# eggsbenedicto/DiffusionRenderer-ComfyUI

Hardware: AMD Instinct MI355X
Metric: denoising_steps_per_sec (higher is better)
Workload: dtype bf16; 1 GPU; inverse pass, 57f x 576 x 1024 clip: EDM Euler step = 1 DiT forward (D=4096, 28 blocks, 32 heads) over S=18432 tokens, guidance 0; parallelism=sp1 (token bands; self-attention exchange: none), weights=random-init (hash generator), 7.2e9 params bf16

## Files before the change

diffusionrenderer-comfyui_amd/csrc/attention.hip:

```cpp
#include <stdlib.h>
#include "drn_common.h"
#include "drn_launchers.h"
#include "mx_quant.h"

#ifndef ATT_EPI_LDS
#define ATT_EPI_LDS 1
#endif
#ifndef ATT_PRIO
#define ATT_PRIO 1
#endif
#ifndef ATT_ABL
#define ATT_ABL 0
#endif
#ifndef ATT_DIAG
#define ATT_DIAG 0
#endif
#ifndef ATT_DMA_IN_S
#define ATT_DMA_IN_S 0
#endif
static_assert(ATT_DMA_IN_S == 0, "ATT_DMA_IN_S > 0 reads clamped K/V rows for tile nt-2: fix S_REQ's offsets first");
#ifndef ATT_PTR
#define ATT_PTR 1
#endif
#ifndef ATT_TIE
// ... 490 lines not shown
    if (oq)
        attention_combine_kernel<true><<<grid, dim3(256), 0, st>>>(opart, mlpart, (bf16_t*)o, nsplit, batch, heads, Sq, ldo, bso,
                                                                   scale_log2e, (uint8_t*)oq, (uint8_t*)os, mx_bs);
    else
        attention_combine_kernel<false><<<grid, dim3(256), 0, st>>>(opart, mlpart, (bf16_t*)o, nsplit, batch, heads, Sq, ldo, bso,
                                                                    scale_log2e, nullptr, nullptr, 0);
}

#ifndef ATT_DEFAULT_SHAPE16
#define ATT_DEFAULT_SHAPE16 1
#endif
static int g_att16 = -1;
extern "C" void drn_attention_force_shape16(int on) { g_att16 = on; }

static bool attention_shape16() {
    static int env16 = -1;
    if (env16 < 0) {
        const char* e = getenv("DRN_ATT16");
        env16 = e ? (e[0] != '0') : ATT_DEFAULT_SHAPE16;
    }
    return (g_att16 >= 0 ? g_att16 : env16) != 0;
}

extern "C" int drn_attention_mx_available(void) { return attention_shape16() ? 1 : 0; }

static int attention_launch(const void* q, const void* k, const void* v, void* o, int batch, int heads, int64_t Sq, int64_t Sk,
                            int64_t ldq, int64_t ldk, int64_t ldv, int64_t ldo, int64_t bsq, int64_t bsk, int64_t bsv,
                            int64_t bso, float scale, int nsplit, void* workspace, void* stream, void* oq = nullptr,
                            void* os = nullptr) {
    DRN_CHECK_ARG(q && k && v && (o || oq) && batch > 0 && heads > 0 && Sq >= 0 && Sk > 0 && nsplit >= 1);
    DRN_CHECK_ARG(ldq % 8 == 0 && ldk % 8 == 0 && ldv % 8 == 0 && ldo % 8 == 0);
    DRN_CHECK_ARG(bsq % 8 == 0 && bsk % 8 == 0 && bsv % 8 == 0 && bso % 8 == 0);
    DRN_CHECK_ARG(((uintptr_t)q & 15) == 0 && ((uintptr_t)k & 15) == 0 && ((uintptr_t)v & 15) == 0 && ((uintptr_t)o & 15) == 0);
    DRN_CHECK_ARG(ldk > 0 && ldv > 0 && 64 * ldk * 2 < (1ll << 32) && 64 * ldv * 2 < (1ll << 32));
    AttnLaunch L;
    DRN_TRY(drn_attention_prologue(&L, oq, os, attention_shape16(), batch, heads, Sq, Sk, ldo, bso, scale, nsplit, workspace, QROWS, KVT));
    if (Sq == 0) return DRN_OK;
    hipStream_t st = (hipStream_t)stream;
    if (attention_shape16()) {
        drn_attention16_launch(q, k, v, o, heads, Sq, Sk, ldq, ldk, ldv, ldo, bsq, bsk, bsv, bso, L.scale_log2e, (int)L.nqb, L.total,
                               L.nsplit, L.kv_chunk, L.opart, L.mlpart, st, L.nsplit > 1 ? nullptr : oq, os, L.mx_bs);
    } else
    attention_fwd_kernel<<<dim3((unsigned)L.total, 1, 1), dim3(512), 0, st>>>(
        (const bf16_t*)q, (const bf16_t*)k, (const bf16_t*)v, (bf16_t*)o, heads, Sq, Sk, ldq, ldk, ldv, ldo, bsq, bsk,
        bsv, bso, L.scale_log2e, (int)L.nqb, (int)L.total, L.nsplit, L.kv_chunk, L.opart, L.mlpart);
    if (L.nsplit > 1)
        drn_attention_combine_launch(L.opart, L.mlpart, o, L.nsplit, batch, heads, Sq, ldo, bso, L.scale_log2e, oq, os, L.mx_bs, st);
    return drn_launch_status();
}

extern "C" int drn_attention_bf16(const void* q, const void* k, const void* v, void* o, int batch, int heads, int64_t Sq,
                                  int64_t Sk, int64_t ldq, int64_t ldk, int64_t ldv, int64_t ldo, int64_t bsq,
                                  int64_t bsk, int64_t bsv, int64_t bso, float scale, void* stream) {
    DRN_CHECK_ARG(o);
    return attention_launch(q, k, v, o, batch, heads, Sq, Sk, ldq, ldk, ldv, ldo, bsq, bsk, bsv, bso, scale, 1, nullptr, stream);
}

extern "C" int drn_attention_bf16_mx(const void* q, const void* k, const void* v, void* o, void* oq, void* os, int batch, int heads,
                                     int64_t Sq, int64_t Sk, int64_t ldq, int64_t ldk, int64_t ldv, int64_t ldo, int64_t bsq,
                                     int64_t bsk, int64_t bsv, int64_t bso, float scale, void* stream) {
    DRN_CHECK_ARG(oq && os);
    return attention_launch(q, k, v, o, batch, heads, Sq, Sk, ldq, ldk, ldv, ldo, bsq, bsk, bsv, bso, scale, 1, nullptr, stream, oq, os);
}

extern "C" int64_t drn_attention_splitkv_workspace_bytes(int batch, int heads, int64_t Sq, int nsplit) {
    return (int64_t)nsplit * batch * Sq * heads * (128 + 2) * (int64_t)sizeof(float);
}

extern "C" int drn_attention_splitkv_bf16(const void* q, const void* k, const void* v, void* o, int batch, int heads, int64_t Sq,
                                          int64_t Sk, int64_t ldq, int64_t ldk, int64_t ldv, int64_t ldo, int64_t bsq,
                                          int64_t bsk, int64_t bsv, int64_t bso, float scale, int nsplit, void* workspace,
                                          void* stream) {
    DRN_CHECK_ARG(o);
    return attention_launch(q, k, v, o, batch, heads, Sq, Sk, ldq, ldk, ldv, ldo, bsq, bsk, bsv, bso, scale, nsplit, workspace,
                            stream);
}

extern "C" int drn_attention_splitkv_bf16_mx(const void* q, const void* k, const void* v, void* o, void* oq, void* os, int batch,
                                             int heads, int64_t Sq, int64_t Sk, int64_t ldq, int64_t ldk, int64_t ldv, int64_t ldo,
                                             int64_t bsq, int64_t bsk, int64_t bsv, int64_t bso, float scale, int nsplit,
                                             void* workspace, void* stream) {
    DRN_CHECK_ARG(oq && os);
    return attention_launch(q, k, v, o, batch, heads, Sq, Sk, ldq, ldk, ldv, ldo, bsq, bsk, bsv, bso, scale, nsplit, workspace,
                            stream, oq, os);
}
```

diffusionrenderer-comfyui_amd/csrc/attention16.hip:

```cpp
#include "drn_common.h"
#include "drn_launchers.h"
#include "mx_quant.h"

#define QROWS 256
#define KVT 64
#define KBYTES (KVT * 256)
#define NKB 3
#define NVB 4
#ifndef RESCALE_THR
#define RESCALE_THR 6.0f
#endif

typedef const __attribute__((address_space(1))) void* gptr_t;
typedef __attribute__((address_space(3))) void* lptr_t;

template <bool MX>
__global__ __launch_bounds__(512, 2) void attention16_fwd_kernel(
    const bf16_t* __restrict__ Q, const bf16_t* __restrict__ Kp, const bf16_t* __restrict__ Vp, bf16_t* __restrict__ O,
    int heads, int64_t Sq, int64_t Sk_total, int64_t ldq, int64_t ldk, int64_t ldv, int64_t ldo, int64_t bsq, int64_t bsk,
    int64_t bsv, int64_t bso, float scale_log2e, int nqb, int total, int nsplit, int64_t kv_chunk,
    float* __restrict__ Opart, float* __restrict__ MLpart, uint8_t* __restrict__ OQ, uint8_t* __restrict__ OS, int64_t mx_bs) {
    __shared__ __attribute__((aligned(1024))) char smem[(NKB + NVB) * KBYTES];

    const int tid = threadIdx.x;
    const int lane = tid & 63;
    const int wave = __builtin_amdgcn_readfirstlane(tid >> 6);
    const int c = lane & 15, g = lane >> 4;

    int pid;
    {
        const int bid = blockIdx.x;
        const int q = total >> 3, r = total & 7, xcd = bid & 7;
        pid = (xcd < r ? xcd * (q + 1) : r * (q + 1) + (xcd - r) * q) + (bid >> 3);
    }
    const int qb = pid % nqb;
    const int rest = pid / nqb;
    const int split = rest % nsplit;
    const int bh = rest / nsplit;
    const int b = bh / heads, head = bh - b * heads;
    const int64_t q0 = (int64_t)qb * QROWS + wave * 32;
    const int64_t kv_begin = (int64_t)split * kv_chunk;
    const int64_t Sk = min(kv_chunk, Sk_total - kv_begin);

    const bf16_t* Qb = Q + b * bsq + (int64_t)head * 128;
    const bf16_t* Kb = Kp + b * bsk + kv_begin * ldk + (int64_t)head * 128;
    const bf16_t* Vb = Vp + b * bsv + kv_begin * ldv + (int64_t)head * 128;

    bf16x8_t qf[2][4];
#pragma unroll
    for (int qt = 0; qt < 2; ++qt) {
        int64_t qrow = q0 + 16 * qt + c;
        if (qrow > Sq - 1) qrow = Sq - 1;
        const bf16_t* qp = Qb + qrow * ldq + 8 * g;
#pragma unroll
        for (int ks = 0; ks < 4; ++ks) qf[qt][ks] = *reinterpret_cast<const bf16x8_t*>(qp + 32 * ks);
    }
#pragma unroll
    for (int qt = 0; qt < 2; ++qt)
#pragma unroll
        for (int ks = 0; ks < 4; ++ks) asm volatile("" : "+v"(qf[qt][ks]));

    int st_row[2], st_kc[2], st_vc[2];
#pragma unroll
    for (int i = 0; i < 2; ++i) {
        st_row[i] = 4 * (2 * wave + i) + (lane >> 4);
        const int cp = lane & 15;
        st_kc[i] = (cp ^ (st_row[i] & 15)) * 8;
        st_vc[i] = (cp ^ (((st_row[i] & 3) << 1) | (((st_row[i] >> 3) & 1) << 3))) * 8;
    }
    const int dma_off = wave * 2048;
    uint32_t kso[2], vso[2];
#pragma unroll
    for (int i = 0; i < 2; ++i) {
        kso[i] = 2u * (uint32_t)(st_row[i] * (int)ldk + st_kc[i]);
        vso[i] = 2u * (uint32_t)(st_row[i] * (int)ldv + st_vc[i]);
    }
    const int last_rows = (int)(Sk - (int64_t)((Sk - 1) / KVT) * KVT);
#define CLAMP_LAST_TILE()                                                                     \
    do {                                                                                      \
        _Pragma("unroll") for (int i = 0; i < 2; ++i) {                                       \
            const int r_ = min(st_row[i], last_rows - 1);                                     \
            kso[i] = 2u * (uint32_t)(r_ * (int)ldk + st_kc[i]);                               \
            vso[i] = 2u * (uint32_t)(r_ * (int)ldv + st_vc[i]);                               \
// ... 186 lines not shown
                pb[s_][qt] = cv.v;                                                            \
            }                                                                                 \
            if (!ATT16_LSUM_MFMA) l_run[qt] += ps[0] + ps[1];                                 \
        }                                                                                     \
    } while (0)

    const float thr_raw = RESCALE_THR / scale_log2e;
    float m_thr[2] = {-INFINITY, -INFINITY}, mcs[2] = {0.f, 0.f};
    const int nt = (int)((Sk + KVT - 1) / KVT);
    const int grp = wave >> 2;
    if (nt == 1 && last_rows < KVT) CLAMP_LAST_TILE();
    {
        const char* k0_ = reinterpret_cast<const char*>(Kb);
        const char* v0_ = reinterpret_cast<const char*>(Vb);
        DMA_PIECE_AT(0, k0_, v0_, 0, 0); DMA_PIECE_AT(1, k0_, v0_, 0, 0); DMA_PIECE_AT(2, k0_, v0_, 0, 0); DMA_PIECE_AT(3, k0_, v0_, 0, 0);
    }
    const int64_t ktile_bytes = (int64_t)KVT * ldk * 2, vtile_bytes = (int64_t)KVT * ldv * 2;
    if (nt > 1) {
        if (nt == 2 && last_rows < KVT) CLAMP_LAST_TILE();
        const char* k1_ = reinterpret_cast<const char*>(Kb) + ktile_bytes;
        const char* v1_ = reinterpret_cast<const char*>(Vb) + vtile_bytes;
        DMA_PIECE_AT(0, k1_, v1_, 1, 1); DMA_PIECE_AT(1, k1_, v1_, 1, 1); DMA_PIECE_AT(2, k1_, v1_, 1, 1); DMA_PIECE_AT(3, k1_, v1_, 1, 1);
    }
    DMA_WAIT(0);
    BARRIER();
    if (nt == 3 && last_rows < KVT) CLAMP_LAST_TILE();
    if (!ATT16_BAR1 && grp == 1) BARRIER();
    const char* kreq_p = reinterpret_cast<const char*>(Kb) + (int64_t)min(2, nt - 1) * ktile_bytes;
    const char* vreq_p = reinterpret_cast<const char*>(Vb) + (int64_t)min(2, nt - 1) * vtile_bytes;
    int kbuf = 0, vbuf = 0;
    int kreq = 2 % NKB, vreq = 2 % NVB;
#define REQ_PIECE_NOW(P)                                                                      \
    do {                                                                                      \
        if (!(ATT16_ABL & 4)) DMA_PIECE_AT(P, kreq_p, vreq_p, kreq, vreq);                    \
        FENCE();                                                                              \
    } while (0)
#define REQ_PIECE(P) do { if (!ATT16_DMA_IN_S) REQ_PIECE_NOW(P); } while (0)
#define AFTER_REQUESTS(T)                                                                     \
    do {                                                                                      \
        kreq = kreq == NKB - 1 ? 0 : kreq + 1;                                                \
        vreq = vreq == NVB - 1 ? 0 : vreq + 1;                                                \
        if ((T) + 3 == nt - 1 && last_rows < KVT) CLAMP_LAST_TILE();     \
        if (!(ATT16_ABL & 8) && (T) + 3 <= nt - 1) { kreq_p += ktile_bytes; vreq_p += vtile_bytes; }    \
    } while (0)
#define M_QK(T)                                                                               \
    do {                                                                                      \
// ... 112 lines not shown
            const int64_t qr = q0 + row;
            if (!MX) {
                if (qr < Sq) *reinterpret_cast<uint4*>(op + qr * ldo) = v;
            } else {
                uint32_t amax = max(max(mx_amax2(v.x), mx_amax2(v.y)), max(mx_amax2(v.z), mx_amax2(v.w)));
                amax = max(amax, (uint32_t)__shfl_xor((int)amax, 1, 64));
                amax = max(amax, (uint32_t)__shfl_xor((int)amax, 2, 64));
                const int e = mx_block_exp(amax);
                const float inv = mx_inv_scale(e);
                if (qr < Sq) {
                    const int64_t r = b * mx_bs + qr;
                    *reinterpret_cast<uint2*>(OQ + (r * heads + head) * 128 + oc * 8) = make_uint2(mx_pack4(v.x, v.y, inv), mx_pack4(v.z, v.w, inv));
                    if ((oc & 3) == 0) OS[(r * heads + head) * 4 + (oc >> 2)] = (uint8_t)(e + 127);
                    if (O) *reinterpret_cast<uint4*>(op + qr * ldo) = v;
                }
            }
        }
    }
}

void drn_attention16_launch(const void* q, const void* k, const void* v, void* o, int heads, int64_t Sq, int64_t Sk, int64_t ldq,
                            int64_t ldk, int64_t ldv, int64_t ldo, int64_t bsq, int64_t bsk, int64_t bsv, int64_t bso,
                            float scale_log2e, int nqb, int64_t total, int nsplit, int64_t kv_chunk, float* opart, float* mlpart,
                            hipStream_t st, void* oq, void* os, int64_t mx_bs) {
    if (oq)
        attention16_fwd_kernel<true><<<dim3((unsigned)total, 1, 1), dim3(512), 0, st>>>(
            (const bf16_t*)q, (const bf16_t*)k, (const bf16_t*)v, (bf16_t*)o, heads, Sq, Sk, ldq, ldk, ldv, ldo, bsq, bsk, bsv, bso,
            scale_log2e, nqb, (int)total, nsplit, kv_chunk, opart, mlpart, (uint8_t*)oq, (uint8_t*)os, mx_bs);
    else
        attention16_fwd_kernel<false><<<dim3((unsigned)total, 1, 1), dim3(512), 0, st>>>(
            (const bf16_t*)q, (const bf16_t*)k, (const bf16_t*)v, (bf16_t*)o, heads, Sq, Sk, ldq, ldk, ldv, ldo, bsq, bsk, bsv, bso,
            scale_log2e, nqb, (int)total, nsplit, kv_chunk, opart, mlpart, nullptr, nullptr, 0);
}
```

diffusionrenderer-comfyui_amd/csrc/dit_forward.hip:

```cpp
#include "drn_common.h"

static const int kCUs = 256;

static int64_t ceil_div(int64_t a, int64_t b) { return (a + b - 1) / b; }

static int pick_kv_splits(int64_t batch, int64_t heads, int64_t Sq, int64_t Sk, double* cost_out) {
    const int64_t blocks = batch * heads * ((Sq + 255) / 256);
    int best = 1;
    double best_cost = (double)ceil_div(blocks, kCUs);
    const int cand[3] = {2, 4, 8};
    for (int i = 0; i < 3; ++i) {
        const int n = cand[i];
        if (Sk / n < 512) break;
        const double cost = (double)ceil_div(blocks * n, kCUs) * (1.0 / n + 0.04) + 0.06;
        const double lim = (double)ceil_div(blocks, kCUs) * 0.93;
        if (cost < (best_cost < lim ? best_cost : lim)) {
            best = n;
            best_cost = cost;
        }
    }
    if (cost_out) *cost_out = best_cost;
    return best;
}

// ... 245 lines not shown
        }
        const int splits = drn_gemm_mxfp8_splitk_choice(clip_rows(M, rpb), N, K);
        Scope sc(timer(), 0, 2.0 * M * N * K, 1.03 * (M * K + N * K) + 2.0 * M * N * (l.residual ? 2 : 1), (hipStream_t)stream);
        if (c_is_mx) *c_is_mx = l.c_mx.q && l.epi == DRN_EPI_GELU && splits <= 1;
        if (c_is_mx && *c_is_mx) return drn_gemm_mxfp8_gelu_mx(A.q, A.s, l.w, l.sw, l.c_mx.q, l.c_mx.s, M, N, K, rpb, stream);
        if (splits == 0) return drn_gemm_mxfp8(A.q, A.s, l.w, l.sw, l.c, M, N, K, N, l.epi, l.gate, l.residual, ldr, rpb, stream);
        if (splits > 1 && defers(l)) {
            deferred = splits;
            deferred_gate = (const bf16_t*)l.gate;
            return drn_gemm_mxfp8_splitk_partials(A.q, A.s, l.w, l.sw, M, N, K, rpb, splits, a->gemm_ws, stream);
        }
        return drn_gemm_mxfp8_splitk(A.q, A.s, l.w, l.sw, l.c, M, N, K, N, l.epi, l.gate, l.residual, ldr, rpb, splits, a->gemm_ws, stream);
    }

    int linear(const Linear& l, bool* c_is_mx = nullptr) { return a->precision == 1 ? linear_mx(l, c_is_mx) : linear_bf16(l); }

    int self_attention(const drn_dit_sub* sb, bool mx_ops, bool o_mx) {
        const int64_t S = a->S, D = a->D, ld = 3 * D, bs = S * 3 * D;
        const int B = (int)a->B, heads = a->heads;
        const float sm_scale = (float)(1.0 / sqrt(128.0));
        bf16_t* q = (bf16_t*)a->QKV;
        bf16_t* k = q + D;
        bf16_t* v = q + 2 * D;
        uint8_t *mxa = nullptr, *kq = nullptr, *vt = nullptr, *ks = nullptr, *vs = nullptr;
        if (mx_ops) {
            mxa = (uint8_t*)a->mx_attn;
            kq = mxa + al[1], vt = mxa + al[2], ks = mxa + al[4], vs = mxa + al[5];
            DRN_TRY(drn_qk_norm_rope_mx(q, k, sb->qn, sb->kn, a->cos, a->sin, mxa + al[0], mxa + al[3], kq, ks, M, heads, ld, ld, S, 0,
                                        a->eps, 0, stream));
            DRN_TRY(drn_mx_quant_vt(v, vt, vs, B, heads, S, ld, bs, stream));
        } else {
            DRN_TRY(drn_qk_norm_rope(q, k, sb->qn, sb->kn, a->cos, a->sin, M, heads, ld, ld, S, 0, a->eps, stream));
        }
        Scope sc(timer(), 1, 4.0 * B * heads * S * S * 128, (mx_ops ? 1.0 : 2.0) * B * heads * 128 * (4.0 * S), (hipStream_t)stream);
        int64_t plan[6];
        const int n = drn_attention_plan(heads, S, S, plan);
        for (int p = 0; p < n; ++p) {
            const int64_t q0 = plan[3 * p], nq = plan[3 * p + 1] - q0;
            const int ns = (int)plan[3 * p + 2];
            bf16_t* o = o_mx ? nullptr : (bf16_t*)a->O + q0 * D;
            uint8_t* oq = o_mx ? (uint8_t*)a->AQ + q0 * D : nullptr;
            uint8_t* os = o_mx ? (uint8_t*)a->AS + q0 * (D / 32) : nullptr;
            if (mx_ops) {
                const uint8_t* qq = mxa + al[0] + q0 * D;
                const uint8_t* qs = mxa + al[3] + q0 * (D / 32);
                DRN_TRY(ns > 1 ? drn_attention_splitkv_mxfp8(qq, qs, kq, ks, vt, vs, o, oq, os, B, heads, nq, S, S, S, D, S * D, sm_scale, ns,
                                                             a->attn_ws, stream)
                               : drn_attention_mxfp8(qq, qs, kq, ks, vt, vs, o, oq, os, B, heads, nq, S, S, S, D, S * D, sm_scale, stream));
            } else if (o_mx) {
                DRN_TRY(ns > 1 ? drn_attention_splitkv_bf16_mx(q + q0 * ld, k, v, nullptr, oq, os, B, heads, nq, S, ld, ld, ld, D, bs, bs, bs,
                                                               S * D, sm_scale, ns, a->attn_ws, stream)
                               : drn_attention_bf16_mx(q + q0 * ld, k, v, nullptr, oq, os, B, heads, nq, S, ld, ld, ld, D, bs, bs, bs, S * D,
                                                       sm_scale, stream));
            } else {
                DRN_TRY(ns > 1 ? drn_attention_splitkv_bf16(q + q0 * ld, k, v, o, B, heads, nq, S, ld, ld, ld, D, bs, bs, bs, S * D, sm_scale,
                                                            ns, a->attn_ws, stream)
                               : drn_attention_bf16(q + q0 * ld, k, v, o, B, heads, nq, S, ld, ld, ld, D, bs, bs, bs, S * D, sm_scale, stream));
            }
        }
        return DRN_OK;
    }
};

int validate(const drn_dit_forward_args* a, int64_t al[8]) {
    DRN_CHECK_ARG(a && a->struct_bytes == (int64_t)sizeof(drn_dit_forward_args));
    DRN_CHECK_ARG(a->S > 0 && a->B > 0 && a->D > 0 && a->heads > 0 && a->D == (int64_t)a->heads * 128 && a->hidden > 0);
    DRN_CHECK_ARG(a->n_sub >= 0 && (a->n_sub == 0 || a->subs) && a->X && a->H && a->QKV && a->O && a->U && a->Y);
    DRN_CHECK_ARG(a->P && a->w_patch && a->w_final && a->final_shift && a->final_scale && a->shift && a->scale && a->gate);
    const int64_t S = a->S, B = a->B, D = a->D;
    DRN_CHECK_ARG(a->precision == 0 || a->precision == 1);
    int64_t need = drn_dit_forward_gemm_workspace_bytes(B, S, D, a->hidden, a->n_final, a->kpad);
// ... 88 lines not shown
```

diffusionrenderer-comfyui_amd/csrc/drn_launchers.h:

```cpp
#pragma once
#include "drn_common.h"

struct ConvGeom;

void drn_attention_combine_launch(const float* opart, const float* mlpart, void* o, int nsplit, int batch, int heads, int64_t Sq,
                                  int64_t ldo, int64_t bso, float scale_log2e, void* oq, void* os, int64_t mx_bs, hipStream_t st);
void drn_attention16_launch(const void* q, const void* k, const void* v, void* o, int heads, int64_t Sq, int64_t Sk, int64_t ldq,
                            int64_t ldk, int64_t ldv, int64_t ldo, int64_t bsq, int64_t bsk, int64_t bsv, int64_t bso,
                            float scale_log2e, int nqb, int64_t total, int nsplit, int64_t kv_chunk, float* opart, float* mlpart,
                            hipStream_t st, void* oq, void* os, int64_t mx_bs);

int drn_gemm256s_dispatch(const void* A, const void* W, void* C, int64_t M, int64_t N, int64_t K, int64_t lda, int64_t ldw,
                          int64_t ldc, int epilogue, const void* gate, const void* residual, int64_t ldr, int64_t rpb,
                          void* stream, const int64_t* blk);
int drn_gemm256s_partial(const void* A, const void* W, float* partial, int64_t M, int64_t N, int64_t K, int64_t lda, int64_t ldw,
                         int splits, void* stream, bool wring_ok);
int drn_gemm144_dispatch(const void* A, const void* W, void* C, int64_t M, int64_t N, int64_t K, int64_t lda, int64_t ldw,
                         int64_t ldc, int epilogue, const void* gate, const void* residual, int64_t ldr, int64_t rpb,
                         void* stream, const int64_t* blk);
int drn_gemm_tall_dispatch(const void* A, const void* W, void* C, float* partial, int64_t M, int64_t N, int64_t K, int64_t lda,
                           int64_t ldw, int64_t ldc, int epilogue, const void* gate, const void* residual, int64_t ldr,
                           int64_t rpb, int splits, void* stream);
int drn_gemm_splitk_reduce(const void* workspace, int splits, void* C, int64_t M, int64_t N, int64_t ldc, int epilogue,
                           const void* gate, const void* residual, int64_t ldr, int64_t rows_per_batch, void* stream);
int drn_gemm_mx_gelu_mx_launch(const void* A, const void* SA, const void* W, const void* SW, void* CQ, void* CS, int64_t M, int64_t N,
                               int64_t K, void* stream);

bool drn_conv256s_ok(const ConvGeom& g, int C, int N, int64_t ldc, int64_t ldr, bool has_residual, bool out_f32, const void* y,
                     const void* residual);
int drn_conv256s_launch(const void* x, const void* w, const void* bias, void* y, const void* residual, const ConvGeom& g, int C,
                        int N, int64_t ldw, int64_t ldc, int64_t ldr, void* stream);

struct AttnLaunch {
// ... 34 lines not shown
```

diffusionrenderer-comfyui_amd/dit_engine.py:

```python
import ctypes
import math
from typing import Dict, Optional

import torch

from . import native as N
from .host_tables import rope_cos_sin, timestep_sinusoid
from .parallel import ShardPlan, allgather_rows_, alltoall_bands_, alltoall_rows_, group_info, wait_exchange


PRECISIONS = ("bf16", "mxfp8")
ATTENTION_PRECISIONS = ("bf16", "mxfp8")


def _pad_cols(w: torch.Tensor, mult: int) -> torch.Tensor:
    n, k = w.shape
    kp = (k + mult - 1) // mult * mult
    if kp == k:
        return w.contiguous()
    out = torch.zeros((n, kp), dtype=w.dtype, device=w.device)
    out[:, :k] = w
    return out


# ... 430 lines not shown
                a.mx_fused = 1
                a.UQ, a.US = ws["uact"].data_ptr(), ws["uact"].data_ptr() + ws["uact_q_bytes"]
                a.u_act_bytes = ws["uact"].numel()
        if self._amx:
            a.attn_precision = 1
            a.mx_attn, a.mx_attn_bytes = ws["mx_attn"].data_ptr(), ws["mx_attn"].numel()
        return a

    def _fa_local(self, sb, hin, ws, cos, sin, gate, S, B, fusedmx):
        D = self.D
        X, O, QKV = ws["x"], ws["o"], ws["qkv"]
        self._lin(hin, sb["wqkv"], QKV, rows_per_batch=S)
        q, k, v = QKV[:, :D], QKV[:, D:2 * D], QKV[:, 2 * D:]
        amx = self._amx and N.attention_mxfp8_choice(self.heads, S)
        omx = (self._mx_view(ws["act"], ws["act_q_bytes"], X.shape[0], D)
               if fusedmx and (amx or N.attention_mx_available()) else None)
        if amx:
            qm, km, vt, vs = ws["mx_attn_views"]
            N.qk_norm_rope_mx(q, k, sb["qn"], sb["kn"], cos, sin, self.heads, tokens_per_batch=S,
                              write_bf16=self.trace is not None, out_q=qm, out_k=km)
            N.mx_quant_vt(QKV.view(B, S, 3 * D)[:, :, 2 * D:], self.heads, out=(vt, vs))
            oin = N.attention_mxfp8(qm, km, vt, vs, B, S, S, out=None if omx else O.view(B, S, D), out_mx=omx)
        else:
            N.qk_norm_rope(q, k, sb["qn"], sb["kn"], cos, sin, self.heads, tokens_per_batch=S)
            Q3 = QKV.view(B, S, 3 * D)
            oin = N.attention(Q3[:, :, :D], Q3[:, :, D:2 * D], Q3[:, :, 2 * D:], out=None if omx else O.view(B, S, D),
                              heads=self.heads, out_mx=omx)
        self._lin(oin if omx else O, sb["wo"], X, epilogue=N.EPI_GATE_RES, gate=gate, residual=X, rows_per_batch=S)

    def _mlp(self, sb, hin, ws, gate, rows, fusedmx):
        X, U = ws["x"], ws["u"]
        uin = U
        if fusedmx and N.mx_gemm_plan(X.shape[0], U.shape[1], self.D, rows) <= 1:
            uin = N.gemm_mxfp8(hin, sb["w1"], epilogue=N.EPI_GELU, rows_per_batch=rows,
                               out_mx=self._mx_view(ws["uact"], ws["uact_q_bytes"], X.shape[0], U.shape[1]))
        else:
            self._lin(hin, sb["w1"], U, epilogue=N.EPI_GELU, rows_per_batch=rows)
        self._lin(uin, sb["w2"], X, epilogue=N.EPI_GATE_RES, gate=gate, residual=X, rows_per_batch=rows)

    def _run(self, x, cond, mod, modf, addvec, Tp, Hp, Wp, plan):
        D = self.D
        S, rows, world = plan.S, plan.rows, plan.world
        B = x.shape[0]
        cos, sin = self.rope(Tp, Hp, Wp)
        ws = self._workspace(S, rows, B)
        X, Hb, O, Y = ws["x"], ws["h"], ws["o"], ws["y"]
        modB = modfB = gateB = None
        if B > 1:
            modB = mod[:, :2 * D].reshape(-1, 2, 1, D).expand(-1, 2, B, D).contiguous()
            modfB = modf.view(2, 1, D).expand(2, B, D).contiguous()
# ... 67 lines not shown
```

diffusionrenderer-comfyui_amd/native.py:

```python
import ctypes
import os
from ctypes import POINTER, Structure, c_char_p, c_double, c_float, c_int, c_int32, c_int64, c_void_p

import torch

_LIB = None
_LIB_NAME = "libdrn.so"

EPI_NONE, EPI_GELU, EPI_GATE_RES = 0, 1, 2
ACT_NONE, ACT_SILU = 0, 1

_P, _I, _L, _F = c_void_p, c_int, c_int64, c_float

SUB_FA, SUB_CA, SUB_MLP = 0, 1, 2


class DitSub(Structure):
    _fields_ = [("kind", c_int32), ("site", c_int32), ("ca_index", c_int32), ("reserved", c_int32),
                ("w_a", c_void_p), ("w_b", c_void_p), ("qn", c_void_p), ("kn", c_void_p),
                ("s_a", c_void_p), ("s_b", c_void_p)]


class DitForwardArgs(Structure):
    _fields_ = [("struct_bytes", c_int64), ("S", c_int64), ("B", c_int64), ("D", c_int64), ("hidden", c_int64),
# ... 28 lines not shown
    "drn_timer_read": [_P, _I, POINTER(c_int), POINTER(c_float), POINTER(c_double), POINTER(c_double)],
    "drn_abi_version": [],
    "drn_error_string": [_I],
    "drn_gemm_bf16": [_P, _P, _P, _L, _L, _L, _L, _L, _L, _I, _P, _P, _L, _L, _P],
    "drn_gemm_bf16_blocked": [_P, _P, _P, _L, _L, _L, _L, _L, _L, _I, _P, _P, _L, _L, _L, _L, _L, _L, _P],
    "drn_gemm_bf16_splitk": [_P, _P, _P, _L, _L, _L, _L, _L, _L, _I, _P, _P, _L, _L, _I, _P, _P],
    "drn_gemm_splitk_workspace_bytes": [_L, _L, _I],
    "drn_gemm_bf16_f32out": [_P, _P, _P, _L, _L, _L, _L, _L, _P],
    "drn_gemm_bf16_splitk_partials": [_P, _P, _L, _L, _L, _L, _L, _L, _I, _P, _P],
    "drn_splitk_gate_res_ln_modulate": [_P, _I, _P, _P, _P, _P, _P, _P, _L, _L, _L, _F, _P],
    "drn_gemm_splitk_choice": [_L, _L, _L],
    "drn_gemm_tile_choice": [_L, _L],
    "drn_gemm_force_tile": [_I],
    "drn_gemm_force_res_prefetch": [_I],
    "drn_gemm_tall_force_shape": [_I],
    "drn_mx_quant_bf16": [_P, _L, _L, _L, _P, _P, _P],
    "drn_mx_quant_calls": [_I],
    "drn_gemm_mxfp8_gelu_mx": [_P, _P, _P, _P, _P, _P, _L, _L, _L, _L, _P],
    "drn_ln_modulate_mx": [_P, _P, _P, _P, _P, _P, _P, _L, _L, _L, _F, _P],
    "drn_splitk_gate_res_ln_modulate_mx": [_P, _I, _P, _P, _P, _P, _P, _P, _P, _P, _L, _L, _L, _F, _P],
    "drn_attention_bf16_mx": [_P, _P, _P, _P, _P, _P, _I, _I, _L, _L, _L, _L, _L, _L, _L, _L, _L, _L, _F, _P],
    "drn_attention_splitkv_bf16_mx": [_P, _P, _P, _P, _P, _P, _I, _I, _L, _L, _L, _L, _L, _L, _L, _L, _L, _L, _F, _I, _P, _P],
    "drn_attention_mx_available": [],
    "drn_attention_mxfp8_params": [POINTER(c_int), POINTER(c_float), POINTER(c_int)],
    "drn_attention_mxfp8_choice": [_I, _L],
    "drn_attention_mxfp8_force": [_I],
    "drn_qk_norm_rope_mx": [_P, _P, _P, _P, _P, _P, _P, _P, _P, _P, _L, _I, _L, _L, _L, _L, _F, _I, _P],
    "drn_mx_quant_vt": [_P, _P, _P, _I, _I, _L, _L, _L, _P],
    "drn_attention_mxfp8": [_P, _P, _P, _P, _P, _P, _P, _P, _P, _I, _I, _L, _L, _L, _L, _L, _L, _F, _P],
    "drn_attention_splitkv_mxfp8": [_P, _P, _P, _P, _P, _P, _P, _P, _P, _I, _I, _L, _L, _L, _L, _L, _L, _F, _I, _P, _P],
    "drn_dit_forward_mx_attn_bytes": [_L, _L, _L],
    "drn_dit_forward_mx_attn_layout": [_L, _L, _L, POINTER(c_int64)],
    "drn_gemm_mxfp8": [_P, _P, _P, _P, _P, _L, _L, _L, _L, _I, _P, _P, _L, _L, _P],
    "drn_gemm_mxfp8_splitk_choice": [_L, _L, _L],
    "drn_gemm_mxfp8_splitk": [_P, _P, _P, _P, _P, _L, _L, _L, _L, _I, _P, _P, _L, _L, _I, _P, _P],
    "drn_gemm_mxfp8_splitk_partials": [_P, _P, _P, _P, _L, _L, _L, _L, _I, _P, _P],
    "drn_gemm_mxfp8_force_small_m": [_I],
    "drn_gemm_mxfp8_tall_force_shape": [_I],
    "drn_gemv_bf16": [_P, _P, _P, _L, _L, _I, _I, _L, _L, _L, _L, _L, _P, _L, _L, _P, _L, _L, _I, _P],
    "drn_ln_modulate": [_P, _P, _P, _P, _P, _L, _L, _L, _F, _P],
    "drn_ln_force_kernel": [_I],
    "drn_bcast_add": [_P, _P, _L, _L, _L, _P],
    "drn_permute_021": [_P, _P, _L, _L, _L, _P],
    "drn_rmsnorm": [_P, _P, _P, _L, _L, _F, _P],
    "drn_qk_norm_rope": [_P, _P, _P, _P, _P, _P, _L, _I, _L, _L, _L, _L, _F, _P],
    "drn_attention_bf16": [_P, _P, _P, _P, _I, _I, _L, _L, _L, _L, _L, _L, _L, _L, _L, _L, _F, _P],
    "drn_attention_splitkv_bf16": [_P, _P, _P, _P, _I, _I, _L, _L, _L, _L, _L, _L, _L, _L, _L, _L, _F, _I, _P, _P],
    "drn_attention_splitkv_workspace_bytes": [_I, _I, _L, _I],
    "drn_attention_force_shape16": [_I],
    "drn_patchify_concat": [_P, _P, _P, _I, _I, _I, _I, _I, _I, _I, _I, _I, _L, _P],
    "drn_unpatchify": [_P, _L, _P, _I, _I, _I, _I, _I, _I, _I, _P],
    "drn_edm_scale_input": [_P, _P, _L, _F, _P],
    "drn_edm_step": [_P, _P, _P, _L, _F, _F, _F, _F, _P],
    "drn_cfg_combine": [_P, _P, _P, _L, _F, _P],
    "drn_postprocess_u8": [_P, _P, _I, _I, _I, _I, _I, _P],
}
_RESTYPES = {"drn_error_string": c_char_p, "drn_attention_splitkv_workspace_bytes": c_int64,
             "drn_gemm_splitk_workspace_bytes": c_int64, "drn_dit_forward_gemm_workspace_bytes": c_int64,
             "drn_dit_forward_attn_workspace_bytes": c_int64, "drn_dit_forward_mx_act_bytes": c_int64,
             "drn_dit_forward_mx_u_bytes": c_int64, "drn_mx_quant_calls": c_int64, "drn_dit_forward_mx_attn_bytes": c_int64,
             "drn_dit_forward_mx_gemm_workspace_bytes": c_int64, "drn_dit_forward_args_bytes": c_int64, "drn_dit_sub_bytes": c_int64, "drn_timer_create": c_void_p, "drn_timer_destroy": None,
             "drn_ln_force_kernel": None, "drn_attention_force_shape16": None}


def library_path() -> str:
    return os.path.join(os.path.dirname(os.path.abspath(__file__)), _LIB_NAME)


def load_library():
    global _LIB
    if _LIB is not None:
        return _LIB
    path = library_path()
    if not os.path.exists(path):
        raise RuntimeError(f"{path} not found: build it with `python __graft_entry__.py` (hipcc --offload-arch=gfx950); "
                           "there is no CPU / eager fallback for the hot path")
    lib = ctypes.CDLL(path)
    for name, argtypes in SIGNATURES.items():
        fn = getattr(lib, name)
        fn.argtypes = argtypes
        fn.restype = _RESTYPES.get(name, c_int)
    if lib.drn_abi_version() != 1:
        raise RuntimeError("libdrn.so ABI version mismatch")
    if lib.drn_dit_forward_args_bytes() != ctypes.sizeof(DitForwardArgs) or lib.drn_dit_sub_bytes() != ctypes.sizeof(DitSub):
        raise RuntimeError("libdrn.so: drn_dit_forward_args / drn_dit_sub layout differs from the ctypes mirror in native.py")
# ... 385 lines not shown
        oq, osc = mx.q.view(B, Sq, HD), mx.scales.view(B, Sq, HD // 32)
        ldo, bso = HD, Sq * HD
    else:
        if out is None:
            out = torch.empty((B, Sq, HD), dtype=torch.bfloat16, device=device)
        ldo, bso = out.stride(1), out.stride(0)
    if scale is None:
        scale = 1.0 / (128 ** 0.5)
    plan = attention_plan(1, H, Sq, Sk) if kv_splits is None else [(0, Sq, int(kv_splits))]
    t0 = _TIMER.begin("attention") if _TIMER is not None else None
    lib = load_library()
    for q0, q1, ns in plan:
        extra = ()
        if ns > 1:
            nbytes = lib.drn_attention_splitkv_workspace_bytes(B, H, q1 - q0, ns)
            extra = (ns, _split_workspace((device, nbytes), nbytes, grow=False).data_ptr())
        launch(q0, q1 - q0, _ptr(out[:, q0:q1]) if out is not None else None, _ptr(oq[:, q0:q1]) if mx is not None else None,
               _ptr(osc[:, q0:q1]) if mx is not None else None, ldo, bso, scale, extra)
    if t0 is not None:
        _TIMER.end("attention", t0, 4.0 * B * H * Sq * Sk * 128, byte_factor * B * H * 128 * (2 * Sq + 2 * Sk))
    return out if mx is None else mx


def attention(q, k, v, out=None, heads=None, scale=None, kv_splits=None, out_mx=None):
    _bf16(q, k, v, out)
    B, Sq, HD = q.shape
    Sk = k.shape[1]
    H = heads if heads else HD // 128
    assert HD == H * 128 and q.stride(2) == 1 and k.stride(2) == 1 and v.stride(2) == 1
    if out_mx is not None and not attention_mx_available():
        raise RuntimeError("attention(out_mx=): the 32x32x16 body is selected and has no MX epilogue (drn.h)")
    lib = load_library()

    def launch(q0, n, o, oq, osc, ldo, bso, scale, extra):
        name = "drn_attention" + ("_splitkv" if extra else "") + "_bf16" + ("_mx" if oq is not None else "")
        outs = (o,) if oq is None else (o, oq, osc)
        _check(getattr(lib, name)(_ptr(q[:, q0:q0 + n]), _ptr(k), _ptr(v), *outs, B, H, n, Sk, q.stride(1), k.stride(1), v.stride(1),
                                  ldo, q.stride(0), k.stride(0), v.stride(0), bso, scale, *extra, _stream()), name)

    return _attention_tail(launch, B, H, Sq, Sk, q.device, out, out_mx, scale, kv_splits, 2.0)


def attention_mxfp8_params():
    kt, thr, pe = c_int(), c_float(), c_int()
    _check(load_library().drn_attention_mxfp8_params(kt, thr, pe), "drn_attention_mxfp8_params")
    return kt.value, thr.value, pe.value


def attention_mxfp8_choice(heads, S) -> bool:
    return bool(load_library().drn_attention_mxfp8_choice(heads, S))


def attention_mxfp8_force(on: int) -> int:
    return int(load_library().drn_attention_mxfp8_force(on))


def qk_norm_rope_mx(q, k, wq, wk, cos, sin, heads, tokens_per_batch=None, pos_offset=0, eps=1e-6, write_bf16=False,
                    out_q=None, out_k=None):
# ... 119 lines not shown
```

include/drn.h:

```cpp
#ifndef DRN_H
#define DRN_H

#include <stdint.h>

#ifdef __cplusplus
extern "C" {
#endif

#define DRN_OK 0
#define DRN_EINVAL (-1)

#define DRN_ABI_VERSION 1

#define DRN_EPI_NONE 0
#define DRN_EPI_GELU 1
#define DRN_EPI_GATE_RES 2

#define DRN_ACT_NONE 0
#define DRN_ACT_SILU 1

int drn_abi_version(void);
const char* drn_error_string(int code);

int drn_gemm_bf16(const void* A, const void* W, void* C, int64_t M, int64_t N, int64_t K,
// ... 75 lines not shown
                       int64_t bsq, int64_t bsk, int64_t bsv, int64_t bso,
                       float scale, void* stream);

void drn_attention_force_shape16(int on);

int drn_attention_splitkv_bf16(const void* q, const void* k, const void* v, void* o,
                               int batch, int heads, int64_t Sq, int64_t Sk,
                               int64_t ldq, int64_t ldk, int64_t ldv, int64_t ldo,
                               int64_t bsq, int64_t bsk, int64_t bsv, int64_t bso,
                               float scale, int nsplit, void* workspace, void* stream);
int64_t drn_attention_splitkv_workspace_bytes(int batch, int heads, int64_t Sq, int nsplit);

int drn_attention_bf16_mx(const void* q, const void* k, const void* v, void* o, void* oq, void* os,
                          int batch, int heads, int64_t Sq, int64_t Sk,
                          int64_t ldq, int64_t ldk, int64_t ldv, int64_t ldo,
                          int64_t bsq, int64_t bsk, int64_t bsv, int64_t bso,
                          float scale, void* stream);
int drn_attention_splitkv_bf16_mx(const void* q, const void* k, const void* v, void* o, void* oq, void* os,
                                  int batch, int heads, int64_t Sq, int64_t Sk,
                                  int64_t ldq, int64_t ldk, int64_t ldv, int64_t ldo,
                                  int64_t bsq, int64_t bsk, int64_t bsv, int64_t bso,
                                  float scale, int nsplit, void* workspace, void* stream);
int drn_attention_mx_available(void);

int drn_attention_mxfp8_params(int* key_tile, float* rescale_thr, int* pexp);
int drn_attention_mxfp8_choice(int heads, int64_t S);
int drn_attention_mxfp8_force(int on);
int drn_qk_norm_rope_mx(void* q, void* k, const void* wq, const void* wk, const void* cos, const void* sin,
                        void* qq, void* qs, void* kq, void* ks,
                        int64_t tokens, int heads, int64_t ldq, int64_t ldk, int64_t tokens_per_batch,
                        int64_t pos_offset, float eps, int write_bf16, void* stream);
int drn_mx_quant_vt(const void* v, void* vt, void* vs, int batch, int heads, int64_t Sk, int64_t ldv, int64_t bsv, void* stream);
int drn_attention_mxfp8(const void* qq, const void* qs, const void* kq, const void* ks, const void* vt, const void* vs,
                        void* o, void* oq, void* os, int batch, int heads, int64_t Sq, int64_t Sk,
                        int64_t q_bs, int64_t k_bs, int64_t ldo, int64_t bso, float scale, void* stream);
int drn_attention_splitkv_mxfp8(const void* qq, const void* qs, const void* kq, const void* ks, const void* vt, const void* vs,
                                void* o, void* oq, void* os, int batch, int heads, int64_t Sq, int64_t Sk,
                                int64_t q_bs, int64_t k_bs, int64_t ldo, int64_t bso, float scale,
                                int nsplit, void* workspace, void* stream);

int drn_attention_plan(int heads, int64_t Sq, int64_t Sk, int64_t* plan);

#define DRN_SUB_FA 0
#define DRN_SUB_CA 1
#define DRN_SUB_MLP 2
typedef struct drn_dit_sub {
// ... 103 lines not shown
```

Before: 3.659 steps/s.

## Fuse Q RMSNorm and RoPE into the bf16 attention kernel prologue

Adds a QN template variant of the shape-16 attention kernel that loads raw Q, applies per-head RMS normalisation with weights and rotary embedding in registers (using permlane swaps for the row reduction), and overlaps this with the first K/V DMA. The standalone qk_norm_rope call now only processes K, so Q is no longer read and written back to global memory before attention. It costs extra registers and prologue work in every attention block, and each query tile redoes the normalisation per KV split.

```diff
diff --git a/diffusionrenderer-comfyui_amd/csrc/attention.hip b/diffusionrenderer-comfyui_amd/csrc/attention.hip
--- a/diffusionrenderer-comfyui_amd/csrc/attention.hip
+++ b/diffusionrenderer-comfyui_amd/csrc/attention.hip
@@ -536,12 +536,16 @@
     return (g_att16 >= 0 ? g_att16 : env16) != 0;
 }
 
+static int g_qnorm = -1;
+extern "C" void drn_attention_force_qnorm(int on) { g_qnorm = on; }
+extern "C" int drn_attention_qnorm_available(void) { return attention_shape16() && g_qnorm != 0 ? 1 : 0; }
+
 extern "C" int drn_attention_mx_available(void) { return attention_shape16() ? 1 : 0; }
 
 static int attention_launch(const void* q, const void* k, const void* v, void* o, int batch, int heads, int64_t Sq, int64_t Sk,
                             int64_t ldq, int64_t ldk, int64_t ldv, int64_t ldo, int64_t bsq, int64_t bsk, int64_t bsv,
                             int64_t bso, float scale, int nsplit, void* workspace, void* stream, void* oq = nullptr,
-                            void* os = nullptr) {
+                            void* os = nullptr, const AttnQNorm* qn = nullptr) {
     DRN_CHECK_ARG(q && k && v && (o || oq) && batch > 0 && heads > 0 && Sq >= 0 && Sk > 0 && nsplit >= 1);
     DRN_CHECK_ARG(ldq % 8 == 0 && ldk % 8 == 0 && ldv % 8 == 0 && ldo % 8 == 0);
     DRN_CHECK_ARG(bsq % 8 == 0 && bsk % 8 == 0 && bsv % 8 == 0 && bso % 8 == 0);
@@ -553,7 +557,7 @@
     hipStream_t st = (hipStream_t)stream;
     if (attention_shape16()) {
         drn_attention16_launch(q, k, v, o, heads, Sq, Sk, ldq, ldk, ldv, ldo, bsq, bsk, bsv, bso, L.scale_log2e, (int)L.nqb, L.total,
-                               L.nsplit, L.kv_chunk, L.opart, L.mlpart, st, L.nsplit > 1 ? nullptr : oq, os, L.mx_bs);
+                               L.nsplit, L.kv_chunk, L.opart, L.mlpart, st, L.nsplit > 1 ? nullptr : oq, os, L.mx_bs, qn);
     } else
     attention_fwd_kernel<<<dim3((unsigned)L.total, 1, 1), dim3(512), 0, st>>>(
         (const bf16_t*)q, (const bf16_t*)k, (const bf16_t*)v, (bf16_t*)o, heads, Sq, Sk, ldq, ldk, ldv, ldo, bsq, bsk,
@@ -598,3 +602,16 @@
     return attention_launch(q, k, v, o, batch, heads, Sq, Sk, ldq, ldk, ldv, ldo, bsq, bsk, bsv, bso, scale, nsplit, workspace,
                             stream, oq, os);
 }
+
+extern "C" int drn_attention_bf16_qnorm(const void* q, const void* k, const void* v, void* o, void* oq, void* os, int batch, int heads,
+                                        int64_t Sq, int64_t Sk, int64_t ldq, int64_t ldk, int64_t ldv, int64_t ldo, int64_t bsq,
+                                        int64_t bsk, int64_t bsv, int64_t bso, float scale, int nsplit, void* workspace,
+                                        const void* wq, const void* cos, const void* sin, int64_t pos_offset, float eps,
+                                        void* stream) {
+    DRN_CHECK_ARG(attention_shape16());
+    DRN_CHECK_ARG(wq && (cos == nullptr) == (sin == nullptr) && pos_offset >= 0 && (oq == nullptr) == (os == nullptr));
+    DRN_CHECK_ARG(((uintptr_t)wq & 15) == 0 && ((uintptr_t)cos & 15) == 0 && ((uintptr_t)sin & 15) == 0);
+    const AttnQNorm qn = {wq, cos, sin, pos_offset, eps};
+    return attention_launch(q, k, v, o, batch, heads, Sq, Sk, ldq, ldk, ldv, ldo, bsq, bsk, bsv, bso, scale, nsplit, workspace, stream,
+                            oq, os, &qn);
+}
diff --git a/diffusionrenderer-comfyui_amd/csrc/attention16.hip b/diffusionrenderer-comfyui_amd/csrc/attention16.hip
--- a/diffusionrenderer-comfyui_amd/csrc/attention16.hip
+++ b/diffusionrenderer-comfyui_amd/csrc/attention16.hip
@@ -14,12 +14,13 @@
 typedef const __attribute__((address_space(1))) void* gptr_t;
 typedef __attribute__((address_space(3))) void* lptr_t;
 
-template <bool MX>
+template <bool MX, bool QN>
 __global__ __launch_bounds__(512, 2) void attention16_fwd_kernel(
     const bf16_t* __restrict__ Q, const bf16_t* __restrict__ Kp, const bf16_t* __restrict__ Vp, bf16_t* __restrict__ O,
     int heads, int64_t Sq, int64_t Sk_total, int64_t ldq, int64_t ldk, int64_t ldv, int64_t ldo, int64_t bsq, int64_t bsk,
     int64_t bsv, int64_t bso, float scale_log2e, int nqb, int total, int nsplit, int64_t kv_chunk,
-    float* __restrict__ Opart, float* __restrict__ MLpart, uint8_t* __restrict__ OQ, uint8_t* __restrict__ OS, int64_t mx_bs) {
+    float* __restrict__ Opart, float* __restrict__ MLpart, uint8_t* __restrict__ OQ, uint8_t* __restrict__ OS, int64_t mx_bs,
+    const bf16_t* __restrict__ WQ, const bf16_t* __restrict__ CS, const bf16_t* __restrict__ SN, int64_t pos0, float eps) {
     __shared__ __attribute__((aligned(1024))) char smem[(NKB + NVB) * KBYTES];
 
     const int tid = threadIdx.x;
@@ -47,6 +48,7 @@
     const bf16_t* Vb = Vp + b * bsv + kv_begin * ldv + (int64_t)head * 128;
 
     bf16x8_t qf[2][4];
+    uint4 qn_w[4], qn_cs[2][4], qn_sn[2][4];
 #pragma unroll
     for (int qt = 0; qt < 2; ++qt) {
         int64_t qrow = q0 + 16 * qt + c;
@@ -54,11 +56,25 @@
         const bf16_t* qp = Qb + qrow * ldq + 8 * g;
 #pragma unroll
         for (int ks = 0; ks < 4; ++ks) qf[qt][ks] = *reinterpret_cast<const bf16x8_t*>(qp + 32 * ks);
-    }
-#pragma unroll
-    for (int qt = 0; qt < 2; ++qt)
-#pragma unroll
-        for (int ks = 0; ks < 4; ++ks) asm volatile("" : "+v"(qf[qt][ks]));
+        if (QN && CS) {
+            const int64_t to = (pos0 + qrow) * 128 + 8 * g;
+#pragma unroll
+            for (int ks = 0; ks < 4; ++ks) {
+                qn_cs[qt][ks] = *reinterpret_cast<const uint4*>(CS + to + 32 * ks);
+                qn_sn[qt][ks] = *reinterpret_cast<const uint4*>(SN + to + 32 * ks);
+            }
+        }
+    }
+    if (QN) {
+#pragma unroll
+        for (int ks = 0; ks < 4; ++ks) qn_w[ks] = *reinterpret_cast<const uint4*>(WQ + 32 * ks + 8 * g);
+        __builtin_amdgcn_sched_barrier(0);
+    } else {
+#pragma unroll
+        for (int qt = 0; qt < 2; ++qt)
+#pragma unroll
+            for (int ks = 0; ks < 4; ++ks) asm volatile("" : "+v"(qf[qt][ks]));
+    }
 
     int st_row[2], st_kc[2], st_vc[2];
 #pragma unroll
@@ -291,6 +307,81 @@
         const char* v1_ = reinterpret_cast<const char*>(Vb) + vtile_bytes;
         DMA_PIECE_AT(0, k1_, v1_, 1, 1); DMA_PIECE_AT(1, k1_, v1_, 1, 1); DMA_PIECE_AT(2, k1_, v1_, 1, 1); DMA_PIECE_AT(3, k1_, v1_, 1, 1);
     }
+    if (QN) {
+        FENCE();
+#pragma unroll
+        for (int qt = 0; qt < 2; ++qt) {
+#pragma unroll
+            for (int ks = 0; ks < 4; ++ks) asm volatile("" : "+v"(qf[qt][ks]));
+            union { bf16x8_t f; uint4 u; } cv;
+            float x[4][8];
+#pragma unroll
+            for (int ks = 0; ks < 4; ++ks) {
+                cv.f = qf[qt][ks];
+                unpack8(cv.u, x[ks]);
+            }
+            float sp[2];
+#pragma unroll
+            for (int vl = 0; vl < 2; ++vl) {
+                const float* lo = x[vl];
+                const float* hi = x[vl + 2];
+                float s = 0.f;
+#pragma unroll
+                for (int i = 0; i < 8; ++i) s += lo[i] * lo[i];
+#pragma unroll
+                for (int i = 0; i < 8; ++i) s += hi[i] * hi[i];
+                sp[vl] = s;
+            }
+#pragma unroll
+            for (int vl = 0; vl < 2; ++vl) {
+                const uint32_t u = __float_as_uint(sp[vl]);
+                const auto r = __builtin_amdgcn_permlane16_swap(u, u, false, false);
+                sp[vl] = __uint_as_float(r[0]) + __uint_as_float(r[1]);
+            }
+#pragma unroll
+            for (int vl = 0; vl < 2; ++vl) {
+                const uint32_t u = __float_as_uint(sp[vl]);
+                const auto r = __builtin_amdgcn_permlane32_swap(u, u, false, false);
+                sp[vl] = __uint_as_float(r[0]) + __uint_as_float(r[1]);
+            }
+            const float s = sp[0] + sp[1];
+            const float rinv = 1.0f / sqrtf(s / 128.0f + eps);
+#pragma unroll
+            for (int ks = 0; ks < 4; ++ks) {
+                float w[8];
+                unpack8(qn_w[ks], w);
+#pragma unroll
+                for (int i = 0; i < 8; ++i) x[ks][i] = (x[ks][i] * rinv) * w[i];
+            }
+            if (CS) {
+#define RBF2(A, B) do { const uint32_t w_ = pack_bf2(A, B); A = bflo(w_); B = bfhi(w_); } while (0)
+#pragma unroll
+                for (int vl = 0; vl < 2; ++vl) {
+                    float cl[8], ch[8], sl[8], sh[8];
+                    unpack8(qn_cs[qt][vl], cl);
+                    unpack8(qn_cs[qt][vl + 2], ch);
+                    unpack8(qn_sn[qt][vl], sl);
+                    unpack8(qn_sn[qt][vl + 2], sh);
+#pragma unroll
+                    for (int i = 0; i < 8; ++i) {
+                        float a = x[vl][i], b = x[vl + 2][i];
+                        RBF2(a, b);
+                        float t0 = a * cl[i], t1 = (-b) * sl[i], u0 = b * ch[i], u1 = a * sh[i];
+                        RBF2(t0, t1);
+                        RBF2(u0, u1);
+                        x[vl][i] = t0 + t1;
+                        x[vl + 2][i] = u0 + u1;
+                    }
+                }
+            }
+#pragma unroll
+            for (int ks = 0; ks < 4; ++ks) {
+                cv.u = pack8(x[ks]);
+                qf[qt][ks] = cv.f;
+            }
+        }
+        FENCE();
+    }
     DMA_WAIT(0);
     BARRIER();
     if (nt == 3 && last_rows < KVT) CLAMP_LAST_TILE();
@@ -449,13 +540,20 @@
 void drn_attention16_launch(const void* q, const void* k, const void* v, void* o, int heads, int64_t Sq, int64_t Sk, int64_t ldq,
                             int64_t ldk, int64_t ldv, int64_t ldo, int64_t bsq, int64_t bsk, int64_t bsv, int64_t bso,
                             float scale_log2e, int nqb, int64_t total, int nsplit, int64_t kv_chunk, float* opart, float* mlpart,
-                            hipStream_t st, void* oq, void* os, int64_t mx_bs) {
-    if (oq)
-        attention16_fwd_kernel<true><<<dim3((unsigned)total, 1, 1), dim3(512), 0, st>>>(
-            (const bf16_t*)q, (const bf16_t*)k, (const bf16_t*)v, (bf16_t*)o, heads, Sq, Sk, ldq, ldk, ldv, ldo, bsq, bsk, bsv, bso,
-            scale_log2e, nqb, (int)total, nsplit, kv_chunk, opart, mlpart, (uint8_t*)oq, (uint8_t*)os, mx_bs);
-    else
-        attention16_fwd_kernel<false><<<dim3((unsigned)total, 1, 1), dim3(512), 0, st>>>(
-            (const bf16_t*)q, (const bf16_t*)k, (const bf16_t*)v, (bf16_t*)o, heads, Sq, Sk, ldq, ldk, ldv, ldo, bsq, bsk, bsv, bso,
-            scale_log2e, nqb, (int)total, nsplit, kv_chunk, opart, mlpart, nullptr, nullptr, 0);
+                            hipStream_t st, void* oq, void* os, int64_t mx_bs, const AttnQNorm* qn) {
+    const AttnQNorm none = {nullptr, nullptr, nullptr, 0, 0.f};
+    const AttnQNorm& n = qn ? *qn : none;
+#define LAUNCH16(MX, QN)                                                                                                          \
+    attention16_fwd_kernel<MX, QN><<<dim3((unsigned)total, 1, 1), dim3(512), 0, st>>>(                                            \
+        (const bf16_t*)q, (const bf16_t*)k, (const bf16_t*)v, (bf16_t*)o, heads, Sq, Sk, ldq, ldk, ldv, ldo, bsq, bsk, bsv, bso,  \
+        scale_log2e, nqb, (int)total, nsplit, kv_chunk, opart, mlpart, (uint8_t*)(MX ? oq : nullptr), (uint8_t*)(MX ? os : nullptr), \
+        MX ? mx_bs : 0, (const bf16_t*)n.wq, (const bf16_t*)n.cos, (const bf16_t*)n.sin, n.pos0, n.eps)
+    if (oq) {
+        if (qn) LAUNCH16(true, true);
+        else LAUNCH16(true, false);
+    } else {
+        if (qn) LAUNCH16(false, true);
+        else LAUNCH16(false, false);
+    }
+#undef LAUNCH16
 }
diff --git a/diffusionrenderer-comfyui_amd/csrc/dit_forward.hip b/diffusionrenderer-comfyui_amd/csrc/dit_forward.hip
--- a/diffusionrenderer-comfyui_amd/csrc/dit_forward.hip
+++ b/diffusionrenderer-comfyui_amd/csrc/dit_forward.hip
@@ -291,6 +291,7 @@
         bf16_t* q = (bf16_t*)a->QKV;
         bf16_t* k = q + D;
         bf16_t* v = q + 2 * D;
+        const bool qfold = !mx_ops && drn_attention_qnorm_available() == 1;
         uint8_t *mxa = nullptr, *kq = nullptr, *vt = nullptr, *ks = nullptr, *vs = nullptr;
         if (mx_ops) {
             mxa = (uint8_t*)a->mx_attn;
@@ -298,6 +299,8 @@
             DRN_TRY(drn_qk_norm_rope_mx(q, k, sb->qn, sb->kn, a->cos, a->sin, mxa + al[0], mxa + al[3], kq, ks, M, heads, ld, ld, S, 0,
                                         a->eps, 0, stream));
             DRN_TRY(drn_mx_quant_vt(v, vt, vs, B, heads, S, ld, bs, stream));
+        } else if (qfold) {
+            DRN_TRY(drn_qk_norm_rope(nullptr, k, nullptr, sb->kn, a->cos, a->sin, M, heads, ld, ld, S, 0, a->eps, stream));
         } else {
             DRN_TRY(drn_qk_norm_rope(q, k, sb->qn, sb->kn, a->cos, a->sin, M, heads, ld, ld, S, 0, a->eps, stream));
         }
@@ -316,6 +319,9 @@
                 DRN_TRY(ns > 1 ? drn_attention_splitkv_mxfp8(qq, qs, kq, ks, vt, vs, o, oq, os, B, heads, nq, S, S, S, D, S * D, sm_scale, ns,
                                                              a->attn_ws, stream)
                                : drn_attention_mxfp8(qq, qs, kq, ks, vt, vs, o, oq, os, B, heads, nq, S, S, S, D, S * D, sm_scale, stream));
+            } else if (qfold) {
+                DRN_TRY(drn_attention_bf16_qnorm(q + q0 * ld, k, v, o, oq, os, B, heads, nq, S, ld, ld, ld, D, bs, bs, bs, S * D, sm_scale, ns,
+                                                 ns > 1 ? a->attn_ws : nullptr, sb->qn, a->cos, a->sin, q0, a->eps, stream));
             } else if (o_mx) {
                 DRN_TRY(ns > 1 ? drn_attention_splitkv_bf16_mx(q + q0 * ld, k, v, nullptr, oq, os, B, heads, nq, S, ld, ld, ld, D, bs, bs, bs,
                                                                S * D, sm_scale, ns, a->attn_ws, stream)
diff --git a/diffusionrenderer-comfyui_amd/csrc/drn_launchers.h b/diffusionrenderer-comfyui_amd/csrc/drn_launchers.h
--- a/diffusionrenderer-comfyui_amd/csrc/drn_launchers.h
+++ b/diffusionrenderer-comfyui_amd/csrc/drn_launchers.h
@@ -5,10 +5,15 @@
 
 void drn_attention_combine_launch(const float* opart, const float* mlpart, void* o, int nsplit, int batch, int heads, int64_t Sq,
                                   int64_t ldo, int64_t bso, float scale_log2e, void* oq, void* os, int64_t mx_bs, hipStream_t st);
+struct AttnQNorm {
+    const void *wq, *cos, *sin;
+    int64_t pos0;
+    float eps;
+};
 void drn_attention16_launch(const void* q, const void* k, const void* v, void* o, int heads, int64_t Sq, int64_t Sk, int64_t ldq,
                             int64_t ldk, int64_t ldv, int64_t ldo, int64_t bsq, int64_t bsk, int64_t bsv, int64_t bso,
                             float scale_log2e, int nqb, int64_t total, int nsplit, int64_t kv_chunk, float* opart, float* mlpart,
-                            hipStream_t st, void* oq, void* os, int64_t mx_bs);
+                            hipStream_t st, void* oq, void* os, int64_t mx_bs, const AttnQNorm* qn = nullptr);
 
 int drn_gemm256s_dispatch(const void* A, const void* W, void* C, int64_t M, int64_t N, int64_t K, int64_t lda, int64_t ldw,
                           int64_t ldc, int epilogue, const void* gate, const void* residual, int64_t ldr, int64_t rpb,
diff --git a/diffusionrenderer-comfyui_amd/dit_engine.py b/diffusionrenderer-comfyui_amd/dit_engine.py
--- a/diffusionrenderer-comfyui_amd/dit_engine.py
+++ b/diffusionrenderer-comfyui_amd/dit_engine.py
@@ -476,10 +476,11 @@
             N.mx_quant_vt(QKV.view(B, S, 3 * D)[:, :, 2 * D:], self.heads, out=(vt, vs))
             oin = N.attention_mxfp8(qm, km, vt, vs, B, S, S, out=None if omx else O.view(B, S, D), out_mx=omx)
         else:
-            N.qk_norm_rope(q, k, sb["qn"], sb["kn"], cos, sin, self.heads, tokens_per_batch=S)
+            qfold = self.trace is None and N.attention_qnorm_available()
+            N.qk_norm_rope(None if qfold else q, k, None if qfold else sb["qn"], sb["kn"], cos, sin, self.heads, tokens_per_batch=S)
             Q3 = QKV.view(B, S, 3 * D)
             oin = N.attention(Q3[:, :, :D], Q3[:, :, D:2 * D], Q3[:, :, 2 * D:], out=None if omx else O.view(B, S, D),
-                              heads=self.heads, out_mx=omx)
+                              heads=self.heads, out_mx=omx, q_norm=(sb["qn"], cos, sin, 0, 1e-6) if qfold else None)
         self._lin(oin if omx else O, sb["wo"], X, epilogue=N.EPI_GATE_RES, gate=gate, residual=X, rows_per_batch=S)
 
     def _mlp(self, sb, hin, ws, gate, rows, fusedmx):
diff --git a/diffusionrenderer-comfyui_amd/native.py b/diffusionrenderer-comfyui_amd/native.py
--- a/diffusionrenderer-comfyui_amd/native.py
+++ b/diffusionrenderer-comfyui_amd/native.py
@@ -74,6 +74,9 @@
     "drn_attention_bf16_mx": [_P, _P, _P, _P, _P, _P, _I, _I, _L, _L, _L, _L, _L, _L, _L, _L, _L, _L, _F, _P],
     "drn_attention_splitkv_bf16_mx": [_P, _P, _P, _P, _P, _P, _I, _I, _L, _L, _L, _L, _L, _L, _L, _L, _L, _L, _F, _I, _P, _P],
     "drn_attention_mx_available": [],
+    "drn_attention_bf16_qnorm": [_P, _P, _P, _P, _P, _P, _I, _I, _L, _L, _L, _L, _L, _L, _L, _L, _L, _L, _F, _I, _P, _P, _P, _P, _L, _F, _P],
+    "drn_attention_force_qnorm": [_I],
+    "drn_attention_qnorm_available": [],
     "drn_attention_mxfp8_params": [POINTER(c_int), POINTER(c_float), POINTER(c_int)],
     "drn_attention_mxfp8_choice": [_I, _L],
     "drn_attention_mxfp8_force": [_I],
@@ -112,7 +115,8 @@
              "drn_dit_forward_attn_workspace_bytes": c_int64, "drn_dit_forward_mx_act_bytes": c_int64,
              "drn_dit_forward_mx_u_bytes": c_int64, "drn_mx_quant_calls": c_int64, "drn_dit_forward_mx_attn_bytes": c_int64,
              "drn_dit_forward_mx_gemm_workspace_bytes": c_int64, "drn_dit_forward_args_bytes": c_int64, "drn_dit_sub_bytes": c_int64, "drn_timer_create": c_void_p, "drn_timer_destroy": None,
-             "drn_ln_force_kernel": None, "drn_attention_force_shape16": None}
+             "drn_ln_force_kernel": None, "drn_attention_force_shape16": None,
+             "drn_attention_force_qnorm": None}
 
 
 def library_path() -> str:
@@ -544,8 +548,19 @@
     return out if mx is None else mx
 
 
-def attention(q, k, v, out=None, heads=None, scale=None, kv_splits=None, out_mx=None):
+def attention_qnorm_available() -> bool:
+    return bool(load_library().drn_attention_qnorm_available())
+
+
+def attention_force_qnorm(on: int) -> None:
+    load_library().drn_attention_force_qnorm(int(on))
+
+
+def attention(q, k, v, out=None, heads=None, scale=None, kv_splits=None, out_mx=None, q_norm=None):
     _bf16(q, k, v, out)
+    if q_norm is not None:
+        wq, cos, sin, pos_offset, eps = q_norm
+        _bf16(wq, cos, sin)
     B, Sq, HD = q.shape
     Sk = k.shape[1]
     H = heads if heads else HD // 128
@@ -556,6 +571,13 @@
 
     def launch(q0, n, o, oq, osc, ldo, bso, scale, extra):
         name = "drn_attention" + ("_splitkv" if extra else "") + "_bf16" + ("_mx" if oq is not None else "")
+        if q_norm is not None:
+            name = "drn_attention_bf16_qnorm"
+            _check(lib.drn_attention_bf16_qnorm(_ptr(q[:, q0:q0 + n]), _ptr(k), _ptr(v), o, oq, osc, B, H, n, Sk, q.stride(1), k.stride(1),
+                                                v.stride(1), ldo, q.stride(0), k.stride(0), v.stride(0), bso, scale,
+                                                *(extra if extra else (1, None)), _ptr(wq), _ptr(cos), _ptr(sin), pos_offset + q0, eps,
+                                                _stream()), name)
+            return
         outs = (o,) if oq is None else (o, oq, osc)
         _check(getattr(lib, name)(_ptr(q[:, q0:q0 + n]), _ptr(k), _ptr(v), *outs, B, H, n, Sk, q.stride(1), k.stride(1), v.stride(1),
                                   ldo, q.stride(0), k.stride(0), v.stride(0), bso, scale, *extra, _stream()), name)
diff --git a/include/drn.h b/include/drn.h
--- a/include/drn.h
+++ b/include/drn.h
@@ -121,6 +121,15 @@
                                   int64_t bsq, int64_t bsk, int64_t bsv, int64_t bso,
                                   float scale, int nsplit, void* workspace, void* stream);
 int drn_attention_mx_available(void);
+
+int drn_attention_bf16_qnorm(const void* q, const void* k, const void* v, void* o, void* oq, void* os,
+                             int batch, int heads, int64_t Sq, int64_t Sk,
+                             int64_t ldq, int64_t ldk, int64_t ldv, int64_t ldo,
+                             int64_t bsq, int64_t bsk, int64_t bsv, int64_t bso,
+                             float scale, int nsplit, void* workspace,
+                             const void* wq, const void* cos, const void* sin, int64_t pos_offset, float eps, void* stream);
+void drn_attention_force_qnorm(int on);
+int drn_attention_qnorm_available(void);
 
 int drn_attention_mxfp8_params(int* key_tile, float* rescale_thr, int* pexp);
 int drn_attention_mxfp8_choice(int heads, int64_t S);
```

Result: slower. 3.602 steps/s (-1.6%).
